# zhiqwang/yolort

Hardware: NVIDIA H100
Metric: images/sec end-to-end (letterbox->NMS) (higher is better)
Workload: dtype f16

## Files before the change

### include/yolort_b200.h

```cpp
#ifndef YOLORT_B200_H
#define YOLORT_B200_H

#include <stddef.h>
#include <stdint.h>

#ifdef __cplusplus
extern "C" {
#endif

#define YB_OK 0
#define YB_ERR_INVALID (-1)
#define YB_ERR_CUDA (-2)
#define YB_ERR_WORKSPACE (-3)

#define YB_U8 0
#define YB_F16 1
#define YB_BF16 2
#define YB_F32 3
#define YB_F8E4M3 4

const char* yb_last_error(void);
int yb_abi_version(void);

typedef struct {
// ... 84 lines not shown
  const void* residual;
  int32_t res_cstride;
  int32_t reserved;
  const yb_head_decode* decode;
  const yb_conv_chain* chain;
} yb_op_desc;

#define YB_CONV_FORCE_IM2COL 1
#define YB_CONV_BAND_STEM 2
#define YB_CONV_FORCE_PLANES 4
#define YB_CONV_NO_NSPLIT 8
#define YB_CONV_ONE_CTA 16
#define YB_CONV_NO_TAIL_SPLIT 64
#define YB_CONV_PAIR_N64 128
#define YB_CONV_NO_TEAMS 256
#define YB_CONV_E4M3_F16_OUT 16
#define YB_CONV_E4M3_BF16_OUT 32

int yb_conv_chain_supported(const yb_op_desc* op);

#define YB_CONV_KERNEL_IM2COL 0
#define YB_CONV_KERNEL_PATCH 1
#define YB_CONV_KERNEL_E4M3 2
#define YB_CONV_TILING_ROWS 0
#define YB_CONV_TILING_CLASSIC 1
#define YB_CONV_TILING_WRAP 2
#define YB_CONV_TILING_STRIDE2 3
typedef struct {
  int32_t kernel;
  int32_t block_n;
// ... 3 lines not shown
  int32_t slots;
  int32_t ring;
  int32_t store_cols;
  int32_t store_bufs;
  int32_t groups;
  int32_t resident_ctas;
  int32_t chained;
  int32_t smem_bytes;
  int32_t grid;
  int32_t tiling;
  int32_t m_tiles;
  int32_t work_items;
  int32_t tail_n;
  int32_t tail_tiles;
  int32_t tail_split;
} yb_conv_info;

int yb_conv_config(const yb_op_desc* op, yb_conv_info* info);

typedef struct yb_plan yb_plan;

int yb_plan_create(const yb_op_desc* ops, int n_ops, yb_plan** plan_out);
int yb_plan_run(yb_plan* plan, void* stream);
int yb_plan_run_range(yb_plan* plan, int first, int count, void* stream);
int yb_plan_num_launches(const yb_plan* plan);
int yb_plan_destroy(yb_plan* plan);

#define YB_MAX_LEVELS 4
#define YB_MAX_ANCHORS 4

// ... 370 lines not shown
```

### yolort_b200/_C.py

```python
import ctypes
import itertools
import math
import os
from typing import Dict, List, Optional, Sequence, Tuple

import torch

_HERE = os.path.dirname(os.path.abspath(__file__))
LIB_PATH = os.environ.get("YB_LIB_PATH") or os.path.join(_HERE, "libyolort_b200.so")

YB_U8, YB_F16, YB_BF16, YB_F32, YB_F8E4M3 = 0, 1, 2, 3, 4
YB_LAYOUT_NCHW, YB_LAYOUT_S2D16 = 0, 1
YB_OP_CONV, YB_OP_SPP_POOL, YB_OP_UPSAMPLE2X, YB_OP_ATTENTION, YB_OP_DWCONV, YB_OP_SE, YB_OP_AVGPOOL = 0, 1, 2, 3, 4, 5, 6
YB_OP_QUANTIZE = 7
YB_ACT_NONE, YB_ACT_SILU, YB_ACT_HARDSWISH, YB_ACT_LEAKY01, YB_ACT_RELU = 0, 1, 2, 3, 4
YB_CONV_FORCE_IM2COL, YB_CONV_BAND_STEM, YB_CONV_FORCE_PLANES, YB_CONV_NO_NSPLIT, YB_CONV_ONE_CTA = 1, 2, 4, 8, 16
YB_CONV_NO_TAIL_SPLIT = 64
YB_CONV_PAIR_N64 = 128
YB_CONV_NO_TEAMS = 256
YB_CONV_E4M3_F16_OUT, YB_CONV_E4M3_BF16_OUT = 16, 32
YB_CONV_KERNEL_IM2COL, YB_CONV_KERNEL_PATCH, YB_CONV_KERNEL_E4M3 = 0, 1, 2
PATCH_TILINGS = {1: "classic", 2: "wrap", 3: "stride2"}
YB_MAX_LEVELS, YB_MAX_ANCHORS = 4, 4
NMS_TV_AUTO, NMS_EXACT_PER_CLASS, NMS_OFFSET_TRICK = 0, 1, 2

EXPORTED_SYMBOLS = (
    "yb_last_error",
    "yb_abi_version",
    "yb_letterbox_geometry",
    "yb_letterbox",
    "yb_letterbox_strided",
    "yb_canvas_rescale",
    "yb_scale_coords_params",
    "yb_conv_chain_supported",
# ... 83 lines not shown
    _fields_ = [
        ("weight", ctypes.c_void_p), ("bias", ctypes.c_void_p),
        ("Cout", ctypes.c_int32), ("Cout_pad", ctypes.c_int32), ("K_pad", ctypes.c_int32),
        ("act", ctypes.c_int32),
        ("out", ctypes.c_void_p), ("out_cstride", ctypes.c_int32),
        ("own_C", ctypes.c_int32),
        ("extra", ctypes.c_void_p), ("extra_C", ctypes.c_int32), ("extra_cstride", ctypes.c_int32),
        ("store_first", ctypes.c_int32),
    ]


class ConvInfo(ctypes.Structure):
    _fields_ = [(name, ctypes.c_int32) for name in (
        "kernel", "block_n", "n_tiles", "weights_resident", "tiles_per_pass", "slots", "ring", "store_cols", "store_bufs",
        "groups", "resident_ctas", "chained", "smem_bytes", "grid", "tiling", "m_tiles", "work_items", "tail_n",
        "tail_tiles", "tail_split")]


class HeadDecode(ctypes.Structure):
    _fields_ = [
        ("n_anchors", ctypes.c_int32), ("n_classes", ctypes.c_int32),
        ("level_start", ctypes.c_int32), ("anchors_per_image", ctypes.c_int32),
        ("stride_px", ctypes.c_float), ("anchors_px", ctypes.c_float * 8),
        ("score_thresh", ctypes.c_float),
        ("cap_per_image", ctypes.c_int64),
        ("keys", ctypes.c_void_p), ("boxes", ctypes.c_void_p),
        ("img_count", ctypes.c_void_p), ("img_maxc", ctypes.c_void_p),
    ]


class NmsLayout(ctypes.Structure):
# ... 435 lines not shown
            seen.add(key)
            im.record_stream(stream)
    return out


def conv_chain_supported(op: "OpDesc") -> bool:
    return bool(lib().yb_conv_chain_supported(ctypes.byref(op)))


def conv_config(op: "OpDesc") -> dict:
    info = ConvInfo()
    check(lib().yb_conv_config(ctypes.byref(op), ctypes.byref(info)), "yb_conv_config")
    patch = info.kernel == YB_CONV_KERNEL_PATCH
    cfg = {k: int(getattr(info, k)) for k in ("block_n", "n_tiles", "weights_resident", "tiles_per_pass", "slots", "ring",
                                               "store_cols", "smem_bytes", "grid", "chained", "resident_ctas", "m_tiles",
                                               "work_items", "tail_n", "tail_tiles", "tail_split")}
    cfg["patch_kernel"] = int(patch)
    cfg["e4m3_kernel"] = int(info.kernel == YB_CONV_KERNEL_E4M3)
    cfg["store_bufs" if patch else "epilogue_groups"] = int(info.store_bufs if patch else info.groups)
    pairs = not patch and info.groups == 4 and info.tiles_per_pass == 2
    cfg["layout"] = f"{info.resident_ctas}x{info.groups}" + ("x2" if pairs else "")
    cfg["consumer_groups"] = int(info.groups)
    cfg["ctas_per_sm"] = 2 if cfg["layout"] == "2x2" else 1
    if patch:
        cfg["patch_tiling"] = PATCH_TILINGS[info.tiling]
    return cfg


class Plan:

    def __init__(self, ops: Sequence[OpDesc], device: torch.device):
# ... 790 lines not shown
```

### yolort_b200/csrc/conv3x3_patch_sm90.cu

```cuda
#include <cstdlib>

#include "common.cuh"
#include "conv_epilogue.cuh"
#include "conv_chain.cuh"
#include "conv_sm90.h"

namespace yb {
namespace {

constexpr int kMaxA = 4, kMaxB = 12;
constexpr int kConsumers = 2;
constexpr int kThreads = 128 * (1 + kConsumers);
constexpr int kStageBufBytes = 128 * 128;
constexpr int kMaxBlockN = 128;
constexpr size_t kSmemBudget = 216 * 1024;
constexpr size_t kStaticSmem = (2 * kMaxA + 2 * kMaxB + 2) * 8 + 2 * kMaxBlockN * 4;
constexpr uint32_t kConsumerBar = 1;

struct TileGeom {
  int tile_h, tile_w;
  int x_step;
  int pitch, patch_h;
  int gpr;
  int sbo_rows;
// ... 6 lines not shown
  int block_n, block_k, chunks;
  int a_slots, b_stages, b_resident;
  int pair;
  int s2;
  int band;
  int ctas;
  int teams;
  int store_cols, store_bufs, bias_len;
  int stage_buf_bytes;
  int kk_last;
  TileGeom tg;
  uint32_t a_bytes, a_stride, b_sub_bytes, b_res_bytes;
  const float* bias;
  EpilogueParams ep;
  ChainParams ch;
};

__device__ __forceinline__ void tma_load_tiled_4d(const void* desc, uint64_t* bar, void* smem_dst, int c, int w,
                                                  int h, int n) {
  asm volatile(
      "cp.async.bulk.tensor.4d.shared::cluster.global.mbarrier::complete_tx::bytes"
      " [%0], [%1, {%3, %4, %5, %6}], [%2];" ::"r"(smem_u32(smem_dst)),
      "l"(reinterpret_cast<uint64_t>(desc)), "r"(smem_u32(bar)), "r"(c), "r"(w), "r"(h), "r"(n)
      : "memory");
}
__device__ __forceinline__ void tma_load_tiled_5d(const void* desc, uint64_t* bar, void* smem_dst, int c, int par, int w,
                                                  int h, int n) {
  asm volatile(
      "cp.async.bulk.tensor.5d.shared::cluster.global.mbarrier::complete_tx::bytes"
      " [%0], [%1, {%3, %4, %5, %6, %7}], [%2];" ::"r"(smem_u32(smem_dst)),
// ... 26 lines not shown
    const uint64_t db = desc_lohi(b_lo + 2 * k, b_hi);
    if (mode == 2) {
      wgmma_mma<kBf16, kN>(acc, desc_lohi(((tap % 3) == 1 ? a0 : a1) + 2 * k, a_hi), db, accum);
    } else {
      wgmma_mma<kBf16, kN>(acc, desc_lohi(a0 + 2 * k, a_hi), db, accum);
      if constexpr (kPair) {
        if (mode == 1) wgmma_mma<kBf16, kN>(acc + kN / 2, desc_lohi(a1 + 2 * k, a_hi), db, accum);
      }
    }
  }
}

template <bool kBf16, bool kChain, int kN>
__device__ __forceinline__ void store_tile(const PatchParams& p, const CUtensorMap* tmap_out, const float* acc, const float* s_bias,
                                           const FragRows& fr, int n0, int x0, int y0, int n_img, uint8_t* staging,
                                           int& store_idx, bool issuer, int lane) {
  const int store_cols = p.store_cols;
  for (int c0 = 0; c0 < p.block_n; c0 += store_cols, ++store_idx) {
    uint8_t* buf = staging + (kChain ? (c0 / store_cols) * kStageBufBytes : (p.store_bufs == 2 ? (store_idx & 1) * p.stage_buf_bytes : 0));
    if (!kChain && p.store_bufs == 1) {
      if (issuer) tma_store_wait_read<0>();
      consumer_sync();
    }
    epilogue_box<kBf16, kN>(p.ep, acc, c0, store_cols, s_bias, fr, n0, buf, lane);
    fence_proxy_async_smem();
    if constexpr (!kChain) {
      if (issuer && p.store_bufs == 2) tma_store_wait_read<0>();
    }
    consumer_sync();
    if (issuer) {
      if ((!kChain || p.ch.store_first) && n0 + c0 < p.ep.Cout) tma_store_4d(tmap_out, buf, n0 + c0, x0, y0, n_img);
      tma_store_commit();
    }
  }
}

template <bool kBf16, int kN, int kN2, int kCtas>
__global__ void __launch_bounds__(kThreads, kCtas)
conv3x3_patch_kernel(const __grid_constant__ CUtensorMap tmap_a, const __grid_constant__ CUtensorMap tmap_b,
                     const __grid_constant__ CUtensorMap tmap_out, const __grid_constant__ CUtensorMap tmap_w2,
                     const __grid_constant__ CUtensorMap tmap_x, const __grid_constant__ CUtensorMap tmap_out2,
                     const PatchParams p) {
  constexpr bool kChain = kN2 != 0;
  constexpr bool kPair = kCtas == 1 && kN <= 64;
  constexpr int kTileAcc = kPair ? kN : kN / 2;
  constexpr bool kLean = kCtas == 2;
  constexpr bool kRealloc = kCtas == 2 || kN == 128 || (kChain && kN == 64);
  extern __shared__ uint8_t smem_raw[];
  __shared__ __align__(8) uint64_t a_full[kMaxA], a_empty[kMaxA];
  __shared__ __align__(8) uint64_t b_full[kMaxB], b_empty[kMaxB];
  __shared__ __align__(8) uint64_t x_full;
  __shared__ __align__(8) uint64_t w2_full;
  __shared__ __align__(16) float s_bias[kMaxBlockN];
  __shared__ __align__(16) float s_bias2[kChain ? kMaxBlockN : 4];

  uint8_t* base = reinterpret_cast<uint8_t*>((reinterpret_cast<uintptr_t>(smem_raw) + 1023) & ~static_cast<uintptr_t>(1023));
  uint8_t* a_buf = base;
  uint8_t* b_buf = a_buf + static_cast<size_t>(p.a_slots) * p.a_stride;
  const size_t b_region = p.b_resident ? p.b_res_bytes : static_cast<size_t>(p.b_stages) * p.b_sub_bytes;
  uint8_t* staging = b_buf + b_region;
  uint8_t* w2_res = staging + static_cast<size_t>(p.store_bufs) * p.stage_buf_bytes;
// ... 23 lines not shown
  if constexpr (kRealloc) {
    if (warp < 4) regs_producer<kCtas>();
  }

  if (warp == 0) {
    int ka = 0;
    for (int task = blockIdx.x; task < p.num_tasks; task += gridDim.x) {
      const int m_first = (task / p.n_tiles) * p.pair;
      const int cnt = p.s2 ? 2 : min(p.pair, p.m_tiles - m_first);
      for (int c = 0; c < p.chunks; ++c) {
        for (int j = 0; j < cnt; ++j, ++ka) {
          int n_img, y0, x0;
          tile_coords(p, p.s2 ? m_first : m_first + j, n_img, y0, x0);
          const int s = ka % p.a_slots;
          mbar_wait(&a_empty[s], ((ka / p.a_slots) & 1) ^ 1);
          if (YB_ELECT()) {
            mbar_expect_tx(&a_full[s], p.a_bytes);
            uint8_t* dst = a_buf + static_cast<size_t>(s) * p.a_stride;
            if (p.s2)
              tma_load_tiled_5d(&tmap_a, &a_full[s], dst, c * p.block_k, j, x0 - 1, 2 * y0 - 1, n_img);
            else
              tma_load_tiled_4d(&tmap_a, &a_full[s], dst, c * p.block_k, x0 - 1, y0 - 1, n_img);
          }
        }
      }
    }
    return;
  }
  if (warp == 2) {
    const uint32_t b_bytes = p.block_n * p.block_k * 2;
    if (p.band) {
      if (lane == 0) {
        mbar_expect_tx(&b_full[0], 6 * b_bytes);
        for (int i = 0; i < 6; ++i)
          tma_load_2d(&tmap_b, &b_full[0], b_buf + static_cast<size_t>(i) * p.b_sub_bytes, i * p.block_k, 0);
      }
    } else if (p.b_resident) {
// ... 77 lines not shown
  consumer_sync();
  if (p.b_resident || p.band) mbar_wait(&b_full[0], 0);
  if constexpr (kChain) mbar_wait(&w2_full, 0);

  int ka = 0, kb = 0, store_idx = 0;
  uint32_t xph = 0;
  for (int task = blockIdx.x; task < p.num_tasks; task += gridDim.x) {
    const int m_first = kLean ? task : (task / p.n_tiles) * p.pair;
    const int cnt = p.s2 ? 2 : (kLean ? 1 : min(p.pair, p.m_tiles - m_first));
    const int n0 = kLean ? 0 : (task % p.n_tiles) * p.block_n;
    if (!fixed_n) {
      consumer_sync();
      for (int i = ctid; i < p.block_n; i += 128 * kConsumers) s_bias[i] = (n0 + i < p.bias_len) ? __ldg(p.bias + n0 + i) : 0.f;
    }
    const int tmode = mode == 1 && cnt == 1 ? 0 : mode;
    for (int c = 0; c < p.chunks; ++c) {
      const int sa0 = ka % p.a_slots, sa1 = (ka + 1) % p.a_slots;
      mbar_wait(&a_full[sa0], (ka / p.a_slots) & 1);
      if (cnt == 2) mbar_wait(&a_full[sa1], ((ka + 1) / p.a_slots) & 1);
      const uint32_t a_lo0 = smem_lo16(a_buf + static_cast<size_t>(sa0) * p.a_stride) + a_wg16;
      const uint32_t a_lo1 = smem_lo16(a_buf + static_cast<size_t>(sa1) * p.a_stride) + a_wg16;
      const bool first_chunk = c == 0;
      wgmma_fence();
      if (!kLean && p.band) {
        const uint32_t prow16 = static_cast<uint32_t>(pitch) * row16;
        for (int ky = 0; ky < 3; ++ky) {
          for (int j = 0; j < 6; ++j) {
            const uint32_t al = a_lo0 + ky * prow16 + 6 + 2 * j;
            const uint32_t b_lo = b_res_lo0 + static_cast<uint32_t>(ky * 2 + (j >> 2)) * b_step16 + 2 * (j & 3);
            wgmma_mma<kBf16, kN>(acc, desc_lohi(al, a_hi), desc_lohi(b_lo, b_hi), ky != 0 || j != 0);
          }
        }
        wgmma_commit();
      } else {
        const int kc = c == p.chunks - 1 ? p.kk_last : kk;
        if (kLean || p.b_resident) {
          const uint32_t b_lo_chunk = b_res_lo0 + static_cast<uint32_t>(c * 9) * b_step16;
          for (int tap = 0; tap < 9; ++tap)
            issue_tap<kBf16, kN, kPair>(tmode, tap, kc, first_chunk && tap == 0, acc, a_lo0 + tap_off16(tap), a_lo1 + tap_off16(tap),
                             a_hi, b_lo_chunk + tap * b_step16, b_hi);
          wgmma_commit();
        } else {
          int prev_sb = -1;
          for (int tap = 0; tap < 9; ++tap, ++kb) {
            const int sb = kb % p.b_stages;
            mbar_wait(&b_full[sb], (kb / p.b_stages) & 1);
            issue_tap<kBf16, kN, kPair>(tmode, tap, kc, first_chunk && tap == 0, acc, a_lo0 + tap_off16(tap), a_lo1 + tap_off16(tap),
                             a_hi, b_res_lo0 + static_cast<uint32_t>(sb) * b_step16, b_hi);
            wgmma_commit();
            wgmma_wait<1>();
            if (prev_sb >= 0 && wg_leader) mbar_arrive(&b_empty[prev_sb]);
            prev_sb = sb;
          }
          wgmma_wait<0>();
          if (wg_leader) mbar_arrive(&b_empty[prev_sb]);
        }
      }
      wgmma_wait<0>();
      if (wg_leader) {
        mbar_arrive(&a_empty[sa0]);
        if (cnt == 2) mbar_arrive(&a_empty[sa1]);
      }
      ka += cnt;
    }
    fence_acc<kTileAcc>(acc);
    if (!fixed_n) consumer_sync();

    const int n_tiles_here = kPair && p.pair == 2 ? cnt : 1;
    int x0 = 0, y0 = 0, n_img = 0;
    for (int tsel = 0; tsel < n_tiles_here; ++tsel) {
      tile_coords(p, m_first + tsel, n_img, y0, x0);
#pragma unroll
      for (int rr = 0; rr < 2; ++rr) {
        const int y = y0 + yy[rr], x = x0 + xx[rr];
        fr.ok[rr] = yy[rr] < p.tg.tile_h && y < p.H && x < p.W;
        fr.row[rr] = (static_cast<long long>(n_img) * p.H + y) * p.W + x;
      }
      if constexpr (kChain) {
        if (issuer) {
          tma_store_wait_read<0>();
          if (p.ch.extra_on) {
            mbar_expect_tx(&x_full, p.ch.extra_bytes);
            tma_load_tiled_4d(&tmap_x, &x_full, staging + p.ch.own_chunks * kStageBufBytes, 0, x0, y0, n_img);
          }
        }
        consumer_sync();
      }
      if (tsel == 0)
        store_tile<kBf16, kChain, kN>(p, &tmap_out, acc, s_bias, fr, n0, x0, y0, n_img, staging, store_idx, issuer, lane);
      else if constexpr (kPair)
        store_tile<kBf16, kChain, kN>(p, &tmap_out, acc + kN / 2, s_bias, fr, n0, x0, y0, n_img, staging, store_idx, issuer, lane);
    }
    if constexpr (kChain) {
      if (p.ch.extra_on) {
        mbar_wait(&x_full, xph);
        xph ^= 1u;
      }
      const uint32_t a2_hi = desc_hi(p.ch.own_row_bytes, 8 * p.ch.own_row_bytes);
      const uint32_t x_hi = desc_hi(p.ch.extra_row_bytes, 8 * p.ch.extra_row_bytes);
      const uint32_t w2_lo0 = smem_lo16(w2_res);
      float acc2[kChain ? kN2 / 2 : 8];
      wgmma_fence();
      for (int j = 0; j < p.ch.w2_chunks; ++j) {
        const bool own = j < p.ch.own_chunks;
        const uint32_t rb = own ? p.ch.own_row_bytes : p.ch.extra_row_bytes;
        const uint32_t a_lo = smem_lo16(staging + j * kStageBufBytes) + ((64 * g * rb) >> 4);
// ... 21 lines not shown
    }
  }
  if (issuer) tma_store_wait_all<0>();
}

constexpr int kQuadConsumers = 4;
constexpr int kQuadThreads = 128 * (1 + kQuadConsumers);
constexpr uint32_t kQuadAllBar = 3;
constexpr size_t kQuadStaticSmem = (2 * kMaxA + 2 * kMaxB) * 8 + kMaxBlockN * 4;
constexpr size_t kQuadSmemBudget = 227 * 1024 - kQuadStaticSmem;

template <bool kBf16>
__global__ void __launch_bounds__(kQuadThreads, 1)
conv3x3_patch_quad_kernel(const __grid_constant__ CUtensorMap tmap_a, const __grid_constant__ CUtensorMap tmap_b,
                          const __grid_constant__ CUtensorMap tmap_out, const __grid_constant__ CUtensorMap,
                          const __grid_constant__ CUtensorMap, const __grid_constant__ CUtensorMap, const PatchParams p) {
  constexpr int kN = 128;
  extern __shared__ uint8_t smem_raw[];
  __shared__ __align__(8) uint64_t a_full[kMaxA], a_empty[kMaxA];
  __shared__ __align__(8) uint64_t b_full[kMaxB], b_empty[kMaxB];
  __shared__ __align__(16) float s_bias[kN];

  uint8_t* base = reinterpret_cast<uint8_t*>((reinterpret_cast<uintptr_t>(smem_raw) + 1023) & ~static_cast<uintptr_t>(1023));
  uint8_t* a_buf = base;
  uint8_t* b_buf = a_buf + static_cast<size_t>(p.a_slots) * p.a_stride;
  uint8_t* staging = b_buf + static_cast<size_t>(p.b_stages) * p.b_sub_bytes;

  const int warp = threadIdx.x >> 5, lane = threadIdx.x & 31;
  const int taps_total = 9 * p.chunks;

  if (threadIdx.x == 0) {
// ... 144 lines not shown
    }
  }
  if (issuer) tma_store_wait_all<0>();
}

constexpr uint32_t kTeamAllBar = 3;
constexpr int kTeamMinTasksPerSm = 8;
constexpr size_t kTeamStaticSmem = (2 * kMaxA + 4) * 8 + 2 * kMaxBlockN * 4;
constexpr size_t kTeamSmemBudget = 227 * 1024 - kTeamStaticSmem;

template <bool kBf16, int kN, int kN2>
__global__ void __launch_bounds__(kQuadThreads, 1)
conv3x3_patch_team_kernel(const __grid_constant__ CUtensorMap tmap_a, const __grid_constant__ CUtensorMap tmap_b,
                          const __grid_constant__ CUtensorMap tmap_out, const __grid_constant__ CUtensorMap tmap_w2,
                          const __grid_constant__ CUtensorMap tmap_x, const __grid_constant__ CUtensorMap tmap_out2,
                          const PatchParams p) {
  constexpr bool kChain = kN2 != 0;
  constexpr bool kBand = !kChain;
  constexpr int kTailChunks = kN2 == 128 ? 2 : 1;
  static_assert(kBand ? kN == 128 : kN == 64, "team instances: the stem (N = 128) or a chain after N = 64");
  extern __shared__ uint8_t smem_raw[];
  __shared__ __align__(8) uint64_t a_full[kMaxA], a_empty[kMaxA];
  __shared__ __align__(8) uint64_t b_full, w2_full;
  __shared__ __align__(8) uint64_t x_full[2];
  __shared__ __align__(16) float s_bias[kN];
  __shared__ __align__(16) float s_bias2[kChain ? kN2 : 4];

  uint8_t* base = reinterpret_cast<uint8_t*>((reinterpret_cast<uintptr_t>(smem_raw) + 1023) & ~static_cast<uintptr_t>(1023));
  uint8_t* a_buf = base;
  uint8_t* b_buf = a_buf + static_cast<size_t>(p.a_slots) * p.a_stride;
  uint8_t* staging = b_buf + p.b_res_bytes;
  uint8_t* w2_res = staging + 4 * kStageBufBytes;

  const int warp = threadIdx.x >> 5, lane = threadIdx.x & 31;
// ... 3 lines not shown
    tma_prefetch_desc(&tmap_b);
    tma_prefetch_desc(&tmap_out);
    for (int s = 0; s < p.a_slots; ++s) {
      mbar_init(&a_full[s], 1);
      mbar_init(&a_empty[s], 2);
    }
    mbar_init(&b_full, 1);
    mbar_init(&w2_full, 1);
    mbar_init(&x_full[0], 1);
    mbar_init(&x_full[1], 1);
    mbar_fence_init();
  }
  __syncthreads();
  if (warp != 2) asm volatile("griddepcontrol.wait;" ::: "memory");
  asm volatile("griddepcontrol.launch_dependents;" ::: "memory");
  if (warp < 4) asm volatile("setmaxnreg.dec.sync.aligned.u32 24;\n" ::: "memory");

  if (warp == 0) {
    int ka = 0;
    for (int task = blockIdx.x; task < p.num_tasks; task += gridDim.x) {
      int n_img, y0, x0;
      tile_coords(p, task, n_img, y0, x0);
      for (int c = 0; c < p.chunks; ++c, ++ka) {
        const int s = ka % p.a_slots;
        mbar_wait(&a_empty[s], ((ka / p.a_slots) & 1) ^ 1);
        if (YB_ELECT()) {
          mbar_expect_tx(&a_full[s], p.a_bytes);
          tma_load_tiled_4d(&tmap_a, &a_full[s], a_buf + static_cast<size_t>(s) * p.a_stride, c * p.block_k, x0 - 1,
                            y0 - 1, n_img);
        }
      }
    }
    return;
  }
  if (warp == 2) {
    if (lane == 0) {
      const uint32_t b_bytes = p.block_n * p.block_k * 2;
      if constexpr (kChain) {
        tma_prefetch_desc(&tmap_w2);
        tma_prefetch_desc(&tmap_out2);
        if (p.ch.extra_on) tma_prefetch_desc(&tmap_x);
        mbar_expect_tx(&w2_full, p.ch.w2_chunks * p.ch.n2 * p.ch.w2_row_bytes);
        for (int j = 0; j < p.ch.w2_chunks; ++j)
          tma_load_2d(&tmap_w2, &w2_full, w2_res + j * p.ch.w2_sub_bytes, j * (p.ch.w2_row_bytes >> 1), 0);
// ... 25 lines not shown
  fr.loc[1] = fr.loc[0] + 8;
  uint8_t* team_staging = staging + static_cast<size_t>(team) * 2 * kStageBufBytes;
  float acc[kN / 2];

  for (int i = ctid; i < kN; i += 128 * kQuadConsumers) s_bias[i] = (i < p.bias_len) ? __ldg(p.bias + i) : 0.f;
  if constexpr (kChain) {
    for (int i = ctid; i < kN2; i += 128 * kQuadConsumers) s_bias2[i] = (i < p.ch.bias2_len) ? __ldg(p.ch.bias2 + i) : 0.f;
  }
  named_bar_sync(kTeamAllBar, 128 * kQuadConsumers);
  mbar_wait(&b_full, 0);
  if constexpr (kChain) mbar_wait(&w2_full, 0);

  uint32_t xph = 0;
  for (int task = blockIdx.x + team * gridDim.x, ka = team * p.chunks; task < p.num_tasks;
       task += 2 * gridDim.x, ka += 2 * p.chunks) {
    {
      const uint32_t row_bytes = p.block_k * 2;
      const uint32_t sbo = p.tg.sbo_rows * row_bytes;
      const uint32_t a_wg16 = (8 * sbo * half) >> 4;
      const uint32_t row16 = row_bytes >> 4;
      const uint32_t a_hi = desc_hi(row_bytes, sbo);
      const uint32_t b_hi = desc_hi(row_bytes, 8 * row_bytes);
      const uint32_t b_lo0 = smem_lo16(b_buf);
      const uint32_t b_step16 = p.b_sub_bytes >> 4;
      if constexpr (kChain) {
#pragma unroll
        for (int i = 0; i < kN / 2; ++i) acc[i] = 0.f;
      }
      for (int c = 0; c < p.chunks; ++c) {
        const int kq = ka + c;
// ... 11 lines not shown
            }
          }
        } else {
          const uint32_t b_lo_chunk = b_lo0 + static_cast<uint32_t>(c * 9) * b_step16;
          for (int tap = 0; tap < 9; ++tap) {
            const int dy = tap / 3, dx = tap - dy * 3;
            const uint32_t a_tap = a_lo + static_cast<uint32_t>(dy * p.tg.pitch + dx) * row16;
            const uint32_t b_lo = b_lo_chunk + static_cast<uint32_t>(tap) * b_step16;
#pragma unroll
            for (int k = 0; k < 4; ++k)
              wgmma_mma<kBf16, kN>(acc, desc_lohi(a_tap + 2 * k, a_hi), desc_lohi(b_lo + 2 * k, b_hi),
                                   !(c == 0 && tap == 0 && k == 0));
          }
        }
        wgmma_commit();
        wgmma_wait<0>();
        if (wg_leader) mbar_arrive(&a_empty[sa]);
      }
    }
    fence_acc<kN / 2>(acc);

    int n_img, y0, x0;
    tile_coords(p, task, n_img, y0, x0);
#pragma unroll
    for (int rr = 0; rr < 2; ++rr) {
      const int y = y0 + (fr.loc[rr] >> 3), x = x0 + (fr.loc[rr] & 7);
      fr.ok[rr] = y < p.H && x < p.W;
      fr.row[rr] = kBand ? 0 : (static_cast<long long>(n_img) * p.H + y) * p.W + x;
    }
    if constexpr (kBand) {
#pragma unroll
      for (int c0 = 0; c0 < kN; c0 += 64) {
        uint8_t* buf = team_staging + (c0 / 64) * kStageBufBytes;
        epilogue_box<kBf16, kN>(p.ep, acc, c0, 64, s_bias, fr, 0, buf, lane);
        fence_proxy_async_smem();
        if (issuer) tma_store_wait_read<0>();
        named_bar_sync(team_bar, 256);
        if (issuer) {
          if (c0 < p.ep.Cout) tma_store_4d(&tmap_out, buf, c0, x0, y0, n_img);
          tma_store_commit();
        }
      }
    } else {
      if (issuer) {
        tma_store_wait_read<0>();
        if (p.ch.extra_on) {
          mbar_expect_tx(&x_full[team], p.ch.extra_bytes);
          tma_load_tiled_4d(&tmap_x, &x_full[team], team_staging + p.ch.own_chunks * kStageBufBytes, 0, x0, y0, n_img);
        }
      }
      named_bar_sync(team_bar, 256);
      epilogue_box<kBf16, kN>(p.ep, acc, 0, p.store_cols, s_bias, fr, 0, team_staging, lane);
      fence_proxy_async_smem();
      named_bar_sync(team_bar, 256);
      if (issuer) {
        if (p.ch.store_first) tma_store_4d(&tmap_out, team_staging, 0, x0, y0, n_img);
        tma_store_commit();
      }
      if (p.ch.extra_on) {
        mbar_wait(&x_full[team], xph);
        xph ^= 1u;
      }
      const uint32_t a2_hi = desc_hi(p.ch.own_row_bytes, 8 * p.ch.own_row_bytes);
      const uint32_t x_hi = desc_hi(p.ch.extra_row_bytes, 8 * p.ch.extra_row_bytes);
      const uint32_t w2_lo0 = smem_lo16(w2_res);
      float acc2[kChain ? kN2 / 2 : 8];
      wgmma_fence();
#pragma unroll
      for (int j = 0; j < kTailChunks; ++j) {
        const bool own = j == 0;
        const uint32_t rb = own ? p.ch.own_row_bytes : p.ch.extra_row_bytes;
        const uint32_t a_lo = smem_lo16(team_staging + j * kStageBufBytes) + ((64 * half * rb) >> 4);
#pragma unroll
        for (int k = 0; k < 4; ++k)
// ... 17 lines not shown
        if (issuer) tma_store_wait_read<0>();
        named_bar_sync(team_bar, 256);
        if (issuer) {
          if (c0 < p.ch.ep2.Cout) tma_store_4d(&tmap_out2, buf, c0, x0, y0, n_img);
          tma_store_commit();
        }
      }
    }
  }
  if (issuer) tma_store_wait_all<0>();
}

}

using PatchKernelFn = void (*)(const CUtensorMap, const CUtensorMap, const CUtensorMap, const CUtensorMap, const CUtensorMap,
                               const CUtensorMap, const PatchParams);

static bool quad_plan(const PatchParams& kp) { return kp.pair == 2 && !kp.s2 && kp.block_n == 128; }

static bool four_groups(const PatchParams& kp) { return quad_plan(kp) || kp.teams; }

template <bool kBf16>
PatchKernelFn select_patch_kernel_t(const PatchParams& kp) {
  if (quad_plan(kp)) return conv3x3_patch_quad_kernel<kBf16>;
  if (kp.teams) {
    if (kp.band) return conv3x3_patch_team_kernel<kBf16, 128, 0>;
    return kp.ch.n2 == 64 ? conv3x3_patch_team_kernel<kBf16, 64, 64> : conv3x3_patch_team_kernel<kBf16, 64, 128>;
  }
  if (kp.ctas == 2) {
    if (kp.ch.on) return kp.block_n == 32 && kp.ch.n2 == 64 ? conv3x3_patch_kernel<kBf16, 32, 64, 2> : nullptr;
    switch (kp.block_n) {
// ... 205 lines not shown
    YB_REQUIRE(kp.b_stages >= 2, "patch conv: not enough shared memory for the weight ring of four consumer warpgroups");
  } else {
    kp.a_slots = (kp.pair == 2 || kp.s2) ? 3 : 2;
    size_t rem = avail - static_cast<size_t>(kp.a_slots) * kp.a_stride;
    if (rem >= static_cast<size_t>(kp.a_stride) + 6 * kp.b_sub_bytes) {
      kp.a_slots += 1;
      rem -= kp.a_stride;
    }
    int b_st = static_cast<int>(rem / kp.b_sub_bytes);
    kp.b_stages = b_st > kMaxB ? kMaxB : b_st;
    if (kp.b_stages < 2) {
      set_error("patch conv: not enough shared memory for the weight ring (block_n=%d)", block_n);
      return YB_ERR_INVALID;
    }
  }
  YB_REQUIRE(kp.a_slots >= 2, "patch conv: fewer than two patch slots fit in shared memory (block_n=%d)", block_n);
  YB_REQUIRE(!kp.teams || kp.a_slots % (2 * kp.chunks) == 0, "patch conv: %d patch slots do not divide between two teams",
             kp.a_slots);
  kp.ep.Cout = d.Cout;
  kp.ep.act = d.act;
  kp.ep.residual = d.residual;
  kp.ep.res_cstride = d.res_cstride;
  kp.bias = d.bias;
  const int max_grid = ctas * sms;
  grid = dim3(kp.num_tasks < max_grid ? kp.num_tasks : max_grid, 1, 1);
  YB_REQUIRE(!(kp.b_resident && n_tiles > 1) || grid.x % n_tiles == 0, "patch conv: N-split grid %u not a multiple of %d", grid.x, n_tiles);
  const size_t b_region = kp.b_resident ? kp.b_res_bytes : static_cast<size_t>(kp.b_stages) * kp.b_sub_bytes;
  const size_t smem = static_cast<size_t>(kp.a_slots) * kp.a_stride + b_region + staging_ns + chain_bytes + 1024;
  const size_t cap = quad ? kQuadSmemBudget : (kp.teams ? kTeamSmemBudget : budget);
  YB_REQUIRE(smem <= cap, "patch conv: %zu bytes of shared memory needed, %zu available", smem, cap);
// ... 14 lines not shown
    info->weights_resident = kp.b_resident;
    info->tiles_per_pass = kp.pair;
    info->slots = kp.a_slots;
    info->ring = kp.b_resident ? 0 : kp.b_stages;
    info->store_cols = kp.store_cols;
    info->store_bufs = kp.store_bufs;
    info->groups = four_groups(kp) ? kQuadConsumers : kConsumers;
    info->resident_ctas = kp.ctas;
    info->chained = kp.ch.on;
    info->smem_bytes = static_cast<int>(smem);
    info->grid = static_cast<int>(grid.x);
    info->tiling = kp.s2 ? YB_CONV_TILING_STRIDE2 : (kp.tg.x_step == 24 ? YB_CONV_TILING_WRAP : YB_CONV_TILING_CLASSIC);
    info->m_tiles = kp.m_tiles;
    info->work_items = kp.num_tasks;
    info->tail_n = kp.ch.n2;
  }
  return rc;
}

struct PatchConvOp final : ConvOp {
  CUtensorMap tmap_a, tmap_b, tmap_out, tmap_w2, tmap_x, tmap_out2;
  PatchParams kp;
  PatchKernelFn fn = nullptr;
  dim3 grid;
  size_t smem_bytes;
  int launch(cudaStream_t stream) const override {
    YB_CHECK_CUDA(launch_pdl(fn, grid, dim3(four_groups(kp) ? kQuadThreads : kThreads), smem_bytes, stream, tmap_a, tmap_b,
                             tmap_out, tmap_w2, tmap_x, tmap_out2, kp));
    return YB_OK;
  }
};

int patch_conv_create(const yb_op_desc& d, ConvOp** out) {
  PatchConvOp* op = new PatchConvOp();
  PatchParams& kp = op->kp;
  int rc = conv_validate(d);
  if (rc == YB_OK) rc = patch_conv_configure(d, kp, op->grid, op->smem_bytes);
  const TileGeom& tg = kp.tg;
  const CUtensorMapDataType dt = kp.ep.is_bf16 ? CU_TENSOR_MAP_DATA_TYPE_BFLOAT16 : CU_TENSOR_MAP_DATA_TYPE_FLOAT16;
  const uint32_t bk = kp.block_k;
  if (rc == YB_OK && kp.s2) {
    const cuuint64_t dims[5] = {static_cast<cuuint64_t>(d.Cin), 2, static_cast<cuuint64_t>(d.W / 2),
                                static_cast<cuuint64_t>(d.H), static_cast<cuuint64_t>(d.N)};
// ... 12 lines not shown
    rc = tmap_matrix(&op->tmap_b, "patch conv weights", dt, d.weight, ktot, d.Cout_pad, ktot, bk, kp.block_n,
                     CU_TENSOR_MAP_L2_PROMOTION_L2_256B);
  const cuuint64_t out_px[3] = {static_cast<cuuint64_t>(d.Wo), static_cast<cuuint64_t>(d.Ho), static_cast<cuuint64_t>(d.N)};
  auto out_view = [&](CUtensorMap* map, const char* what, const void* base, int C, int cstride, uint32_t box_c,
                      CUtensorMapL2promotion l2) {
    const cuuint64_t dims[4] = {static_cast<cuuint64_t>(C), out_px[0], out_px[1], out_px[2]};
    const cuuint32_t box[4] = {box_c, static_cast<cuuint32_t>(tg.tile_w), static_cast<cuuint32_t>(tg.tile_h), 1};
    return tmap_tiled(map, what, dt, base, 4, dims, cstride, box, l2);
  };
  if (rc == YB_OK)
    rc = out_view(&op->tmap_out, "patch conv output", d.out, d.Cout, d.out_cstride, kp.store_cols,
                  CU_TENSOR_MAP_L2_PROMOTION_NONE);
  op->tmap_w2 = op->tmap_b;
  op->tmap_x = op->tmap_a;
  op->tmap_out2 = op->tmap_out;
  if (rc == YB_OK && kp.ch.on) {
    const yb_conv_chain& c = *d.chain;
    const uint32_t kc = kp.ch.w2_row_bytes / 2;
    rc = tmap_matrix(&op->tmap_w2, "patch conv chained tail weights", dt, c.weight, c.K_pad, c.Cout_pad, c.K_pad, kc,
                     kp.ch.n2, CU_TENSOR_MAP_L2_PROMOTION_L2_256B);
    if (rc == YB_OK && kp.ch.extra_on)
      rc = out_view(&op->tmap_x, "patch conv chained tail extra operand", c.extra, c.extra_C, c.extra_cstride, kc,
                    CU_TENSOR_MAP_L2_PROMOTION_L2_128B);
    if (rc == YB_OK)
      rc = out_view(&op->tmap_out2, "patch conv chained tail output", c.out, c.Cout, c.out_cstride, 64,
                    CU_TENSOR_MAP_L2_PROMOTION_NONE);
  }
  if (rc == YB_OK) {
    op->fn = select_patch_kernel(kp);
    const bool quad = four_groups(kp);
// ... 26 lines not shown
```

### yolort_b200/csrc/conv_epilogue.cuh

```cuda
#pragma once
#include "common.cuh"

namespace yb {

struct EpilogueParams {
  int Cout;
  int act, is_bf16;
  const void* residual;
  int res_cstride;
};

__device__ __forceinline__ float ex2_approx(float x) {
  float y;
  asm("ex2.approx.ftz.f32 %0, %1;" : "=f"(y) : "f"(x));
  return y;
}
__device__ __forceinline__ float rcp_approx(float x) {
  float y;
  asm("rcp.approx.ftz.f32 %0, %1;" : "=f"(y) : "f"(x));
  return y;
}
__device__ __forceinline__ float silu(float v) { return v * rcp_approx(1.0f + ex2_approx(v * -1.4426950408889634f)); }

template <bool kBf16>
// ... 31 lines not shown
  if (p.act == YB_ACT_SILU) {
    v0 = silu(v0);
    v1 = silu(v1);
  } else if (p.act == YB_ACT_HARDSWISH) {
    v0 = v0 * fminf(fmaxf(v0 + 3.0f, 0.f), 6.0f) * (1.0f / 6.0f);
    v1 = v1 * fminf(fmaxf(v1 + 3.0f, 0.f), 6.0f) * (1.0f / 6.0f);
  } else if (p.act >= YB_ACT_LEAKY01) {
    const float slope = p.act == YB_ACT_LEAKY01 ? 0.1f : 0.f;
    v0 = fmaxf(v0, v0 * slope);
    v1 = fmaxf(v1, v1 * slope);
  }
}

template <bool kBf16>
__device__ __forceinline__ uint32_t epilogue_pair(const EpilogueParams& p, float v0, float v1, long long row, bool row_ok,
                                                  int gcol) {
  act_pair(p, v0, v1);
  if (p.residual != nullptr && row_ok && gcol < p.Cout) {
    const uint16_t* r = reinterpret_cast<const uint16_t*>(p.residual) + row * p.res_cstride + gcol;
    const float2 f = unpack2<kBf16>(__ldg(reinterpret_cast<const unsigned int*>(r)));
    v0 += f.x;
    v1 += f.y;
  }
  return pack2<kBf16>(v0, v1);
}

template <bool kBf16, int kN>
__device__ __forceinline__ void epilogue_box(const EpilogueParams& p, const float* acc, int c0, int cols,
                                             const float* __restrict__ s_bias, const FragRows& fr, int n0, uint8_t* buf,
                                             int lane) {
  const int row_bytes = cols * 2;
  const int q2 = 2 * (lane & 3);
#pragma unroll
  for (int j = 0; j < kN / 8; ++j) {
    if (8 * j >= c0 && 8 * j < c0 + cols) {
      const int col = 8 * j + q2;
      const float b0 = s_bias[col], b1 = s_bias[col + 1];
#pragma unroll
      for (int rr = 0; rr < 2; ++rr) {
        const uint32_t o = epilogue_pair<kBf16>(p, acc[4 * j + 2 * rr] + b0, acc[4 * j + 2 * rr + 1] + b1,
                                                fr.row[rr], fr.ok[rr], n0 + col);
        const int r = fr.loc[rr];
        *reinterpret_cast<uint32_t*>(buf + r * row_bytes + swizzle_chunk(r, (col - c0) >> 3, row_bytes) * 16 +
                                     ((col - c0) & 7) * 2) = o;
      }
    }
  }
}

}
```

### yolort_b200/csrc/conv_sm90.cu

```cuda
#include <cstdlib>

#include "common.cuh"
#include "conv_sm90.h"
#include "conv_epilogue.cuh"
#include "conv_chain.cuh"
#include "decode_common.cuh"

namespace yb {

namespace {

constexpr int kMaxStages = 12;
__host__ __device__ constexpr int tile_rows(int groups) { return 64 * groups; }
__host__ __device__ constexpr int cta_threads(int groups) { return 128 * (1 + groups); }
__host__ __device__ constexpr int stage_buf_bytes(int groups) { return tile_rows(groups) * 128; }
constexpr int kStageBufs = 2;
constexpr int kMaxBlockN = 256;
constexpr size_t kSmemBudget = 216 * 1024;
constexpr size_t kStaticSmem = (2 * kMaxStages + 2) * 8 + 2 * kMaxBlockN * 4;
constexpr uint32_t kConsumerBar = 1;

struct ConvKernelParams {
  int M, block_n, block_k;
  int ksize, chunks, num_k_iters;
// ... 787 lines not shown
    default: return conv_wgmma_kernel<kBf16, 256, false, 0, 1>;
  }
}
ConvKernelFn select_conv_kernel(const ConvKernelParams& kp) {
  return kp.ep.is_bf16 ? select_conv_kernel_t<true>(kp) : select_conv_kernel_t<false>(kp);
}

}

static int conv_plan(const yb_op_desc& d, int ctas, int groups, ConvKernelParams& kp, dim3& grid, size_t& smem_bytes);
static void conv_team_plan(ConvKernelParams& kp, size_t& smem_bytes);
static void conv_quad_plan(ConvKernelParams& kp, dim3& grid, size_t& smem_bytes);

int conv_validate(const yb_op_desc& d) {
  YB_REQUIRE(d.dtype == YB_F16 || d.dtype == YB_BF16, "conv: dtype must be f16 or bf16");
  YB_REQUIRE((d.reserved & ~(31 | YB_CONV_NO_TAIL_SPLIT | YB_CONV_PAIR_N64 | YB_CONV_NO_TEAMS)) == 0,
             "conv: reserved bits 5 and 9 and up must be zero, got 0x%x",
             d.reserved);
  YB_REQUIRE(d.ksize >= 1 && d.ksize <= 7 && d.stride >= 1 && d.stride <= 2, "conv: ksize/stride");
  YB_REQUIRE(d.act >= YB_ACT_NONE && d.act <= YB_ACT_RELU, "conv: unknown activation %d", d.act);
  YB_REQUIRE(d.Cin % 8 == 0 && d.in_cstride % 8 == 0 && d.in_cstride >= d.Cin,
             "conv: Cin/in_cstride must be multiples of 8 (16-byte TMA granularity), got %d/%d", d.Cin,
             d.in_cstride);
  YB_REQUIRE(d.Cout % 8 == 0 && d.out_cstride % 8 == 0 && d.out_cstride >= d.Cout,
             "conv: Cout/out_cstride must be multiples of 8, got %d/%d", d.Cout, d.out_cstride);
  YB_REQUIRE(d.Cin_pad % 16 == 0 && d.Cin_pad >= d.Cin, "conv: Cin_pad must be a multiple of 16");
  YB_REQUIRE(d.Cout_pad % 16 == 0 && d.Cout_pad >= d.Cout, "conv: Cout_pad must be a multiple of 16");
  YB_REQUIRE((reinterpret_cast<uintptr_t>(d.in) & 15) == 0 && (reinterpret_cast<uintptr_t>(d.out) & 15) == 0 &&
                 (reinterpret_cast<uintptr_t>(d.weight) & 15) == 0,
             "conv: tensors must be 16-byte aligned");
  YB_REQUIRE(d.residual == nullptr ||
                 ((reinterpret_cast<uintptr_t>(d.residual) & 15) == 0 && d.res_cstride % 8 == 0),
// ... 287 lines not shown
```

Baseline: 9595.

## Prefetch residual shortcut tile via TMA into shared memory for patch conv epilogue

In the 3x3 patch conv kernels (two-CTA lean chain path and team kernels), the residual tile is now loaded by TMA alongside the last input chunk or the chain's extra tile, instead of being read with per-element __ldg in the epilogue. The epilogue then reads the residual from swizzled shared memory. The chain's extra-input TMA load is also issued earlier, right after the last wgmma commit, so it overlaps the epilogue. The cost is extra shared memory per slot, which can mean fewer slots, plus changed register limits and more complex barrier and slot-release logic. A new flag turns the path off.

```diff
diff --git a/include/yolort_b200.h b/include/yolort_b200.h
--- a/include/yolort_b200.h
+++ b/include/yolort_b200.h
@@ -122,6 +122,7 @@
 #define YB_CONV_NO_TAIL_SPLIT 64
 #define YB_CONV_PAIR_N64 128
 #define YB_CONV_NO_TEAMS 256
+#define YB_CONV_SHORTCUT_LDG 512
 #define YB_CONV_E4M3_F16_OUT 16
 #define YB_CONV_E4M3_BF16_OUT 32
 
@@ -155,6 +156,7 @@
   int32_t tail_n;
   int32_t tail_tiles;
   int32_t tail_split;
+  int32_t shortcut_in_slot;
 } yb_conv_info;
 
 int yb_conv_config(const yb_op_desc* op, yb_conv_info* info);
diff --git a/yolort_b200/_C.py b/yolort_b200/_C.py
--- a/yolort_b200/_C.py
+++ b/yolort_b200/_C.py
@@ -18,6 +18,7 @@
 YB_CONV_NO_TAIL_SPLIT = 64
 YB_CONV_PAIR_N64 = 128
 YB_CONV_NO_TEAMS = 256
+YB_CONV_SHORTCUT_LDG = 512
 YB_CONV_E4M3_F16_OUT, YB_CONV_E4M3_BF16_OUT = 16, 32
 YB_CONV_KERNEL_IM2COL, YB_CONV_KERNEL_PATCH, YB_CONV_KERNEL_E4M3 = 0, 1, 2
 PATCH_TILINGS = {1: "classic", 2: "wrap", 3: "stride2"}
@@ -131,7 +132,7 @@
     _fields_ = [(name, ctypes.c_int32) for name in (
         "kernel", "block_n", "n_tiles", "weights_resident", "tiles_per_pass", "slots", "ring", "store_cols", "store_bufs",
         "groups", "resident_ctas", "chained", "smem_bytes", "grid", "tiling", "m_tiles", "work_items", "tail_n",
-        "tail_tiles", "tail_split")]
+        "tail_tiles", "tail_split", "shortcut_in_slot")]
 
 
 class HeadDecode(ctypes.Structure):
@@ -597,7 +598,8 @@
     patch = info.kernel == YB_CONV_KERNEL_PATCH
     cfg = {k: int(getattr(info, k)) for k in ("block_n", "n_tiles", "weights_resident", "tiles_per_pass", "slots", "ring",
                                                "store_cols", "smem_bytes", "grid", "chained", "resident_ctas", "m_tiles",
-                                               "work_items", "tail_n", "tail_tiles", "tail_split")}
+                                               "work_items", "tail_n", "tail_tiles", "tail_split",
+                                               "shortcut_in_slot")}
     cfg["patch_kernel"] = int(patch)
     cfg["e4m3_kernel"] = int(info.kernel == YB_CONV_KERNEL_E4M3)
     cfg["store_bufs" if patch else "epilogue_groups"] = int(info.store_bufs if patch else info.groups)
diff --git a/yolort_b200/csrc/conv3x3_patch_sm90.cu b/yolort_b200/csrc/conv3x3_patch_sm90.cu
--- a/yolort_b200/csrc/conv3x3_patch_sm90.cu
+++ b/yolort_b200/csrc/conv3x3_patch_sm90.cu
@@ -44,6 +44,7 @@
   const float* bias;
   EpilogueParams ep;
   ChainParams ch;
+  uint32_t res_off, res_bytes;
 };
 
 __device__ __forceinline__ void tma_load_tiled_4d(const void* desc, uint64_t* bar, void* smem_dst, int c, int w,
@@ -100,7 +101,7 @@
 template <bool kBf16, bool kChain, int kN>
 __device__ __forceinline__ void store_tile(const PatchParams& p, const CUtensorMap* tmap_out, const float* acc, const float* s_bias,
                                            const FragRows& fr, int n0, int x0, int y0, int n_img, uint8_t* staging,
-                                           int& store_idx, bool issuer, int lane) {
+                                           int& store_idx, bool issuer, int lane, const uint8_t* res_box = nullptr) {
   const int store_cols = p.store_cols;
   for (int c0 = 0; c0 < p.block_n; c0 += store_cols, ++store_idx) {
     uint8_t* buf = staging + (kChain ? (c0 / store_cols) * kStageBufBytes : (p.store_bufs == 2 ? (store_idx & 1) * p.stage_buf_bytes : 0));
@@ -108,7 +109,7 @@
       if (issuer) tma_store_wait_read<0>();
       consumer_sync();
     }
-    epilogue_box<kBf16, kN>(p.ep, acc, c0, store_cols, s_bias, fr, n0, buf, lane);
+    epilogue_box<kBf16, kN>(p.ep, acc, c0, store_cols, s_bias, fr, n0, buf, lane, res_box);
     fence_proxy_async_smem();
     if constexpr (!kChain) {
       if (issuer && p.store_bufs == 2) tma_store_wait_read<0>();
@@ -126,11 +127,12 @@
 conv3x3_patch_kernel(const __grid_constant__ CUtensorMap tmap_a, const __grid_constant__ CUtensorMap tmap_b,
                      const __grid_constant__ CUtensorMap tmap_out, const __grid_constant__ CUtensorMap tmap_w2,
                      const __grid_constant__ CUtensorMap tmap_x, const __grid_constant__ CUtensorMap tmap_out2,
-                     const PatchParams p) {
+                     const PatchParams p, const __grid_constant__ CUtensorMap tmap_res) {
   constexpr bool kChain = kN2 != 0;
   constexpr bool kPair = kCtas == 1 && kN <= 64;
   constexpr int kTileAcc = kPair ? kN : kN / 2;
   constexpr bool kLean = kCtas == 2;
+  constexpr bool kResSlot = kChain && kLean;
   constexpr bool kRealloc = kCtas == 2 || kN == 128 || (kChain && kN == 64);
   extern __shared__ uint8_t smem_raw[];
   __shared__ __align__(8) uint64_t a_full[kMaxA], a_empty[kMaxA];
@@ -184,13 +186,15 @@
           tile_coords(p, p.s2 ? m_first : m_first + j, n_img, y0, x0);
           const int s = ka % p.a_slots;
           mbar_wait(&a_empty[s], ((ka / p.a_slots) & 1) ^ 1);
+          const bool res_here = kResSlot && p.res_bytes != 0 && c == p.chunks - 1;
           if (YB_ELECT()) {
-            mbar_expect_tx(&a_full[s], p.a_bytes);
+            mbar_expect_tx(&a_full[s], p.a_bytes + (res_here ? p.res_bytes : 0u));
             uint8_t* dst = a_buf + static_cast<size_t>(s) * p.a_stride;
             if (p.s2)
               tma_load_tiled_5d(&tmap_a, &a_full[s], dst, c * p.block_k, j, x0 - 1, 2 * y0 - 1, n_img);
             else
               tma_load_tiled_4d(&tmap_a, &a_full[s], dst, c * p.block_k, x0 - 1, y0 - 1, n_img);
+            if (res_here) tma_load_tiled_4d(&tmap_res, &a_full[s], dst + p.res_off, 0, x0, y0, n_img);
           }
         }
       }
@@ -298,6 +302,7 @@
       for (int i = ctid; i < p.block_n; i += 128 * kConsumers) s_bias[i] = (n0 + i < p.bias_len) ? __ldg(p.bias + n0 + i) : 0.f;
     }
     const int tmode = mode == 1 && cnt == 1 ? 0 : mode;
+    int res_slot = -1;
     for (int c = 0; c < p.chunks; ++c) {
       const int sa0 = ka % p.a_slots, sa1 = (ka + 1) % p.a_slots;
       mbar_wait(&a_full[sa0], (ka / p.a_slots) & 1);
@@ -324,6 +329,15 @@
             issue_tap<kBf16, kN, kPair>(tmode, tap, kc, first_chunk && tap == 0, acc, a_lo0 + tap_off16(tap), a_lo1 + tap_off16(tap),
                              a_hi, b_lo_chunk + tap * b_step16, b_hi);
           wgmma_commit();
+          if constexpr (kResSlot) {
+            if (issuer && p.ch.extra_on && c == p.chunks - 1) {
+              int xn, xy, xx0;
+              tile_coords(p, m_first, xn, xy, xx0);
+              tma_store_wait_read<0>();
+              mbar_expect_tx(&x_full, p.ch.extra_bytes);
+              tma_load_tiled_4d(&tmap_x, &x_full, staging + p.ch.own_chunks * kStageBufBytes, 0, xx0, xy, xn);
+            }
+          }
         } else {
           int prev_sb = -1;
           for (int tap = 0; tap < 9; ++tap, ++kb) {
@@ -341,7 +355,9 @@
         }
       }
       wgmma_wait<0>();
-      if (wg_leader) {
+      if (kResSlot && p.res_bytes != 0 && c == p.chunks - 1)
+        res_slot = sa0;
+      else if (wg_leader) {
         mbar_arrive(&a_empty[sa0]);
         if (cnt == 2) mbar_arrive(&a_empty[sa1]);
       }
@@ -363,17 +379,26 @@
       if constexpr (kChain) {
         if (issuer) {
           tma_store_wait_read<0>();
-          if (p.ch.extra_on) {
+          if (!kResSlot && p.ch.extra_on) {
             mbar_expect_tx(&x_full, p.ch.extra_bytes);
             tma_load_tiled_4d(&tmap_x, &x_full, staging + p.ch.own_chunks * kStageBufBytes, 0, x0, y0, n_img);
           }
         }
         consumer_sync();
       }
-      if (tsel == 0)
-        store_tile<kBf16, kChain, kN>(p, &tmap_out, acc, s_bias, fr, n0, x0, y0, n_img, staging, store_idx, issuer, lane);
-      else if constexpr (kPair)
+      if (tsel == 0) {
+        const uint8_t* res_box = nullptr;
+        if constexpr (kResSlot) {
+          if (res_slot >= 0) res_box = a_buf + static_cast<size_t>(res_slot) * p.a_stride + p.res_off;
+        }
+        store_tile<kBf16, kChain, kN>(p, &tmap_out, acc, s_bias, fr, n0, x0, y0, n_img, staging, store_idx, issuer, lane,
+                                      res_box);
+      } else if constexpr (kPair) {
         store_tile<kBf16, kChain, kN>(p, &tmap_out, acc + kN / 2, s_bias, fr, n0, x0, y0, n_img, staging, store_idx, issuer, lane);
+      }
+    }
+    if constexpr (kResSlot) {
+      if (res_slot >= 0 && wg_leader) mbar_arrive(&a_empty[res_slot]);
     }
     if constexpr (kChain) {
       if (p.ch.extra_on) {
@@ -425,7 +450,8 @@
 __global__ void __launch_bounds__(kQuadThreads, 1)
 conv3x3_patch_quad_kernel(const __grid_constant__ CUtensorMap tmap_a, const __grid_constant__ CUtensorMap tmap_b,
                           const __grid_constant__ CUtensorMap tmap_out, const __grid_constant__ CUtensorMap,
-                          const __grid_constant__ CUtensorMap, const __grid_constant__ CUtensorMap, const PatchParams p) {
+                          const __grid_constant__ CUtensorMap, const __grid_constant__ CUtensorMap, const PatchParams p,
+                          const __grid_constant__ CUtensorMap) {
   constexpr int kN = 128;
   extern __shared__ uint8_t smem_raw[];
   __shared__ __align__(8) uint64_t a_full[kMaxA], a_empty[kMaxA];
@@ -600,10 +626,12 @@
 conv3x3_patch_team_kernel(const __grid_constant__ CUtensorMap tmap_a, const __grid_constant__ CUtensorMap tmap_b,
                           const __grid_constant__ CUtensorMap tmap_out, const __grid_constant__ CUtensorMap tmap_w2,
                           const __grid_constant__ CUtensorMap tmap_x, const __grid_constant__ CUtensorMap tmap_out2,
-                          const PatchParams p) {
+                          const PatchParams p, const __grid_constant__ CUtensorMap tmap_res) {
   constexpr bool kChain = kN2 != 0;
   constexpr bool kBand = !kChain;
   constexpr int kTailChunks = kN2 == 128 ? 2 : 1;
+  constexpr bool kResStage = kN2 == 64;
+  constexpr bool kResX = kN2 == 128;
   static_assert(kBand ? kN == 128 : kN == 64, "team instances: the stem (N = 128) or a chain after N = 64");
   extern __shared__ uint8_t smem_raw[];
   __shared__ __align__(8) uint64_t a_full[kMaxA], a_empty[kMaxA];
@@ -637,7 +665,12 @@
   __syncthreads();
   if (warp != 2) asm volatile("griddepcontrol.wait;" ::: "memory");
   asm volatile("griddepcontrol.launch_dependents;" ::: "memory");
-  if (warp < 4) asm volatile("setmaxnreg.dec.sync.aligned.u32 24;\n" ::: "memory");
+  if (warp < 4) {
+    if constexpr (kResStage)
+      asm volatile("setmaxnreg.dec.sync.aligned.u32 32;\n" ::: "memory");
+    else
+      asm volatile("setmaxnreg.dec.sync.aligned.u32 24;\n" ::: "memory");
+  }
 
   if (warp == 0) {
     int ka = 0;
@@ -647,10 +680,13 @@
       for (int c = 0; c < p.chunks; ++c, ++ka) {
         const int s = ka % p.a_slots;
         mbar_wait(&a_empty[s], ((ka / p.a_slots) & 1) ^ 1);
+        const bool res_here = kResStage && p.res_bytes != 0 && c == p.chunks - 1;
         if (YB_ELECT()) {
-          mbar_expect_tx(&a_full[s], p.a_bytes);
+          mbar_expect_tx(&a_full[s], p.a_bytes + (res_here ? p.res_bytes : 0u));
           tma_load_tiled_4d(&tmap_a, &a_full[s], a_buf + static_cast<size_t>(s) * p.a_stride, c * p.block_k, x0 - 1,
                             y0 - 1, n_img);
+          if (res_here)
+            tma_load_tiled_4d(&tmap_res, &a_full[s], staging + (2 * (ka & 1) + 1) * kStageBufBytes, 0, x0, y0, n_img);
         }
       }
     }
@@ -706,6 +742,7 @@
   uint32_t xph = 0;
   for (int task = blockIdx.x + team * gridDim.x, ka = team * p.chunks; task < p.num_tasks;
        task += 2 * gridDim.x, ka += 2 * p.chunks) {
+    const bool res_held = kResStage && p.res_bytes != 0;
     {
       const uint32_t row_bytes = p.block_k * 2;
       const uint32_t sbo = p.tg.sbo_rows * row_bytes;
@@ -747,8 +784,19 @@
           }
         }
         wgmma_commit();
+        if constexpr (kChain) {
+          if (issuer && p.ch.extra_on && c == p.chunks - 1) {
+            int xn, xy, xx0;
+            tile_coords(p, task, xn, xy, xx0);
+            const bool res_x = kResX && p.res_bytes != 0;
+            tma_store_wait_read<0>();
+            mbar_expect_tx(&x_full[team], p.ch.extra_bytes + (res_x ? p.res_bytes : 0u));
+            tma_load_tiled_4d(&tmap_x, &x_full[team], team_staging + p.ch.own_chunks * kStageBufBytes, 0, xx0, xy, xn);
+            if (res_x) tma_load_tiled_4d(&tmap_res, &x_full[team], team_staging, 0, xx0, xy, xn);
+          }
+        }
         wgmma_wait<0>();
-        if (wg_leader) mbar_arrive(&a_empty[sa]);
+        if (wg_leader && !(res_held && c == p.chunks - 1)) mbar_arrive(&a_empty[sa]);
       }
     }
     fence_acc<kN / 2>(acc);
@@ -775,22 +823,23 @@
         }
       }
     } else {
-      if (issuer) {
-        tma_store_wait_read<0>();
-        if (p.ch.extra_on) {
-          mbar_expect_tx(&x_full[team], p.ch.extra_bytes);
-          tma_load_tiled_4d(&tmap_x, &x_full[team], team_staging + p.ch.own_chunks * kStageBufBytes, 0, x0, y0, n_img);
-        }
-      }
+      if (issuer) tma_store_wait_read<0>();
       named_bar_sync(team_bar, 256);
-      epilogue_box<kBf16, kN>(p.ep, acc, 0, p.store_cols, s_bias, fr, 0, team_staging, lane);
+      const bool res_x = kResX && p.res_bytes != 0;
+      if (res_x) {
+        mbar_wait(&x_full[team], xph);
+        xph ^= 1u;
+      }
+      const uint8_t* res_box = res_held ? team_staging + kStageBufBytes : (res_x ? team_staging : nullptr);
+      epilogue_box<kBf16, kN>(p.ep, acc, 0, p.store_cols, s_bias, fr, 0, team_staging, lane, res_box);
       fence_proxy_async_smem();
       named_bar_sync(team_bar, 256);
+      if (res_held && wg_leader) mbar_arrive(&a_empty[(ka + p.chunks - 1) % p.a_slots]);
       if (issuer) {
         if (p.ch.store_first) tma_store_4d(&tmap_out, team_staging, 0, x0, y0, n_img);
         tma_store_commit();
       }
-      if (p.ch.extra_on) {
+      if (p.ch.extra_on && !res_x) {
         mbar_wait(&x_full[team], xph);
         xph ^= 1u;
       }
@@ -838,7 +887,7 @@
 }
 
 using PatchKernelFn = void (*)(const CUtensorMap, const CUtensorMap, const CUtensorMap, const CUtensorMap, const CUtensorMap,
-                               const CUtensorMap, const PatchParams);
+                               const CUtensorMap, const PatchParams, const CUtensorMap);
 
 static bool quad_plan(const PatchParams& kp) { return kp.pair == 2 && !kp.s2 && kp.block_n == 128; }
 
@@ -1074,6 +1123,26 @@
       return YB_ERR_INVALID;
     }
   }
+  kp.res_off = kp.res_bytes = 0;
+  if (d.residual != nullptr && kp.ch.on && (ctas == 2 || kp.teams) && !(d.reserved & YB_CONV_SHORTCUT_LDG) &&
+      kp.num_tasks >= kTeamMinTasksPerSm * sms && (reinterpret_cast<uintptr_t>(d.residual) & 15) == 0 &&
+      d.res_cstride % 8 == 0) {
+    const uint32_t box_bytes = static_cast<uint32_t>(tg.tile_w * tg.tile_h * kp.store_cols * 2);
+    if (kp.teams) {
+      if ((!kp.ch.extra_on && kp.ch.n2 == 64 && kp.chunks == 1 && kp.a_slots == 2) || (kp.ch.extra_on && kp.ch.n2 == 128))
+        kp.res_bytes = box_bytes;
+    } else {
+      const uint32_t stride = kp.a_stride + ((static_cast<uint32_t>(128 * kp.store_cols * 2) + 1023u) & ~1023u);
+      int slots = static_cast<int>((avail_ns - b_total) / stride);
+      if (slots > kMaxA) slots = kMaxA;
+      if (slots >= 2) {
+        kp.res_off = kp.a_stride;
+        kp.res_bytes = box_bytes;
+        kp.a_stride = stride;
+        kp.a_slots = slots;
+      }
+    }
+  }
   YB_REQUIRE(kp.a_slots >= 2, "patch conv: fewer than two patch slots fit in shared memory (block_n=%d)", block_n);
   YB_REQUIRE(!kp.teams || kp.a_slots % (2 * kp.chunks) == 0, "patch conv: %d patch slots do not divide between two teams",
              kp.a_slots);
@@ -1118,19 +1187,20 @@
     info->m_tiles = kp.m_tiles;
     info->work_items = kp.num_tasks;
     info->tail_n = kp.ch.n2;
+    info->shortcut_in_slot = kp.res_bytes != 0;
   }
   return rc;
 }
 
 struct PatchConvOp final : ConvOp {
-  CUtensorMap tmap_a, tmap_b, tmap_out, tmap_w2, tmap_x, tmap_out2;
+  CUtensorMap tmap_a, tmap_b, tmap_out, tmap_w2, tmap_x, tmap_out2, tmap_res;
   PatchParams kp;
   PatchKernelFn fn = nullptr;
   dim3 grid;
   size_t smem_bytes;
   int launch(cudaStream_t stream) const override {
     YB_CHECK_CUDA(launch_pdl(fn, grid, dim3(four_groups(kp) ? kQuadThreads : kThreads), smem_bytes, stream, tmap_a, tmap_b,
-                             tmap_out, tmap_w2, tmap_x, tmap_out2, kp));
+                             tmap_out, tmap_w2, tmap_x, tmap_out2, kp, tmap_res));
     return YB_OK;
   }
 };
@@ -1173,6 +1243,10 @@
   op->tmap_w2 = op->tmap_b;
   op->tmap_x = op->tmap_a;
   op->tmap_out2 = op->tmap_out;
+  op->tmap_res = op->tmap_out;
+  if (rc == YB_OK && kp.res_bytes != 0)
+    rc = out_view(&op->tmap_res, "patch conv shortcut", d.residual, d.Cout, d.res_cstride, kp.store_cols,
+                  CU_TENSOR_MAP_L2_PROMOTION_L2_128B);
   if (rc == YB_OK && kp.ch.on) {
     const yb_conv_chain& c = *d.chain;
     const uint32_t kc = kp.ch.w2_row_bytes / 2;
diff --git a/yolort_b200/csrc/conv_epilogue.cuh b/yolort_b200/csrc/conv_epilogue.cuh
--- a/yolort_b200/csrc/conv_epilogue.cuh
+++ b/yolort_b200/csrc/conv_epilogue.cuh
@@ -69,11 +69,11 @@
 
 template <bool kBf16>
 __device__ __forceinline__ uint32_t epilogue_pair(const EpilogueParams& p, float v0, float v1, long long row, bool row_ok,
-                                                  int gcol) {
+                                                  int gcol, const uint32_t* res_s = nullptr) {
   act_pair(p, v0, v1);
   if (p.residual != nullptr && row_ok && gcol < p.Cout) {
     const uint16_t* r = reinterpret_cast<const uint16_t*>(p.residual) + row * p.res_cstride + gcol;
-    const float2 f = unpack2<kBf16>(__ldg(reinterpret_cast<const unsigned int*>(r)));
+    const float2 f = unpack2<kBf16>(res_s != nullptr ? *res_s : __ldg(reinterpret_cast<const unsigned int*>(r)));
     v0 += f.x;
     v1 += f.y;
   }
@@ -83,7 +83,7 @@
 template <bool kBf16, int kN>
 __device__ __forceinline__ void epilogue_box(const EpilogueParams& p, const float* acc, int c0, int cols,
                                              const float* __restrict__ s_bias, const FragRows& fr, int n0, uint8_t* buf,
-                                             int lane) {
+                                             int lane, const uint8_t* res_box = nullptr) {
   const int row_bytes = cols * 2;
   const int q2 = 2 * (lane & 3);
 #pragma unroll
@@ -93,8 +93,14 @@
       const float b0 = s_bias[col], b1 = s_bias[col + 1];
 #pragma unroll
       for (int rr = 0; rr < 2; ++rr) {
+        const uint32_t* res_s = nullptr;
+        if (res_box != nullptr) {
+          const int r = fr.loc[rr];
+          res_s = reinterpret_cast<const uint32_t*>(res_box + r * row_bytes + swizzle_chunk(r, (col - c0) >> 3, row_bytes) * 16 +
+                                                    ((col - c0) & 7) * 2);
+        }
         const uint32_t o = epilogue_pair<kBf16>(p, acc[4 * j + 2 * rr] + b0, acc[4 * j + 2 * rr + 1] + b1,
-                                                fr.row[rr], fr.ok[rr], n0 + col);
+                                                fr.row[rr], fr.ok[rr], n0 + col, res_s);
         const int r = fr.loc[rr];
         *reinterpret_cast<uint32_t*>(buf + r * row_bytes + swizzle_chunk(r, (col - c0) >> 3, row_bytes) * 16 +
                                      ((col - c0) & 7) * 2) = o;
diff --git a/yolort_b200/csrc/conv_sm90.cu b/yolort_b200/csrc/conv_sm90.cu
--- a/yolort_b200/csrc/conv_sm90.cu
+++ b/yolort_b200/csrc/conv_sm90.cu
@@ -825,8 +825,8 @@
 
 int conv_validate(const yb_op_desc& d) {
   YB_REQUIRE(d.dtype == YB_F16 || d.dtype == YB_BF16, "conv: dtype must be f16 or bf16");
-  YB_REQUIRE((d.reserved & ~(31 | YB_CONV_NO_TAIL_SPLIT | YB_CONV_PAIR_N64 | YB_CONV_NO_TEAMS)) == 0,
-             "conv: reserved bits 5 and 9 and up must be zero, got 0x%x",
+  YB_REQUIRE((d.reserved & ~(31 | YB_CONV_NO_TAIL_SPLIT | YB_CONV_PAIR_N64 | YB_CONV_NO_TEAMS | YB_CONV_SHORTCUT_LDG)) == 0,
+             "conv: reserved bits 5 and 10 and up must be zero, got 0x%x",
              d.reserved);
   YB_REQUIRE(d.ksize >= 1 && d.ksize <= 7 && d.stride >= 1 && d.stride <= 2, "conv: ksize/stride");
   YB_REQUIRE(d.act >= YB_ACT_NONE && d.act <= YB_ACT_RELU, "conv: unknown activation %d", d.act);
```

Result: no change. 9641 (median of 6 runs) (+0.5%).
